# StavrosOrf/PoweFlowNet

Measured on AMD Instinct MI355X. Metric: graphs/sec fwd+bwd (train step incl. AdamW), case118v2 batch=128, higher is better.
Workload: dtype f32; 1 GPU; case118v2 (118 buses, 186 branches, synthetic topology) MaskEmbdMultiMPN standard.json (H129 L4 K3 dropout 0.2) training step fwd+MSELoss+bwd+AdamW, fp32; graphs_per_gpu=128, global_batch=128, nodes_per_gpu=15104, directed_edges_per_gpu=47616, parallelism=dp1, launch=hipGraph replay: one graph, undirected_on_device=True

## Files before the change

### poweflownet_amd/csrc/gemm_nt.hip

```cpp
#include <stddef.h>
#include <stdlib.h>
#include <string.h>

#include <algorithm>
#include <type_traits>
#include <vector>

#include "pfn_internal.hpp"

namespace pfn {

constexpr int NT_THREADS = 512;
constexpr int NT_WAVES = NT_THREADS / 64;
constexpr int NCH = 17;
constexpr int KP = 8 * NCH;
constexpr int NT_MAX_PIECES = 16;
constexpr int NT_LDS_BYTES = 160 * 1024;

__global__ __launch_bounds__(256) void pack_weights_kernel(const PackArgs a) {
    if (a.rng_advance && blockIdx.x == 0 && blockIdx.y == 0 && threadIdx.x == 0) a.rng_advance[1] += 1;
    if (a.stamp && blockIdx.x == 0 && blockIdx.y == 0 && threadIdx.x == 0) *a.stamp = a.stamp_value;
    if (a.mask_count > 0) {
        const int64_t nthr = (int64_t)gridDim.x * gridDim.y * blockDim.x;
        for (int64_t i = ((int64_t)blockIdx.y * gridDim.x + blockIdx.x) * blockDim.x + threadIdx.x; i < a.mask_count; i += nthr)
// ... 140 lines not shown
                case 1: wait_a<NCH - 2 + XW>(a_cur[m]); break;
                case 2: wait_a<NCH - 3 + XW>(a_cur[m]); break;
                default: wait_a<NCH - 4 + XW>(a_cur[m]); break;
            }
            const f32x4 av = a_cur[m];
#pragma unroll
            for (int i = 0; i < ((FAST && m == NFAST - 1) ? LS : 4); ++i) {
#pragma unroll
                for (int ct = 0; ct < CT; ++ct) acc[ct] = __builtin_amdgcn_mfma_f32_32x32x2f32(av[i], b[ct][i], acc[ct], 0, 0, 0);
#pragma unroll
                for (int c = 0; c < NR; ++c) racc[c] = fmaf(av[i], r[c][i], racc[c]);
            }
            slice(m);
            if (SLICED) {
#pragma unroll
                for (int c = 0; c < NR; ++c) PFN_OPAQUE(racc[c]);
            }
        }
        if ((m & 3) == 3 || m == NCH - 1) {
#pragma unroll
            for (int mm = m & ~3; mm <= m; ++mm) {
                if (FAST && DIET && mm < NFAST - 1) {
                    vload_x4(a_cur[mm], nbase + (size_t)mm * 8u * nkscale, vlane0);
                } else {
                    const uint32_t kk = min(kh4 + 8u * mm, (uint32_t)nkmax);
                    vload_x4(a_cur[mm], nbase, nvoff + nkscale * kk);
                }
            }
        }
        __builtin_amdgcn_sched_barrier(0);
    }
}

template <int CT, int VAR, bool PAIR = false, bool ILF = false>
__global__ __launch_bounds__(NT_THREADS, 1) void gemm_nt_kernel(const NtArgs a) {
    extern __shared__ __attribute__((aligned(16))) float lds[];
    constexpr int CTE = CT > 0 ? CT : 1;
    const int tid = threadIdx.x, lane = tid & 63;
    const int wave = __builtin_amdgcn_readfirstlane(tid >> 6);
    const int r32 = lane & 31, kh = lane >> 5;
    int bx = blockIdx.x, slice = blockIdx.y;
    {
        const int gx = gridDim.x, ns = gridDim.y, full = gx & ~7;
        const int lin = blockIdx.y * gx + blockIdx.x;
        if (ns > 1 && lin < full * ns) {
            const int chunk = lin / (8 * ns), r = lin - chunk * 8 * ns;
            slice = r >> 3;
            bx = chunk * 8 + (r & 7);
        } else if (ns > 1) {
            const int t = lin - full * ns, tail = gx - full;
            slice = t / tail;
            bx = full + (t - slice * tail);
        }
    }
    const int cg = wave & ((1 << a.cshift) - 1);
    const int rsub = wave >> a.cshift;
    const int rw = NT_WAVES >> a.cshift;
    const int tile0 = slice * a.tps + cg * CT;
    const bool mfma_on = CT > 0 && tile0 < a.nq;
    const bool rem_on = a.remv > 0 && slice == (int)gridDim.y - 1 && cg == 0;
    const int rem_col = 32 * a.nq;
    const int nrt = (a.M + 31) >> 5;
    const int rt_step = gridDim.x * rw;
    int rt = rsub * (int)gridDim.x + bx;

    auto prt = [&](int t) { return a.reverse ? nrt - 1 - t : t; };
    auto a_base = [&](int rt2, int p2) -> const char* {
        return reinterpret_cast<const char*>(a.piece[p2].A + (size_t)prt(rt2) * 32 * a.piece[p2].lda);
    };
// ... 68 lines not shown
    if constexpr (PAIR) {
#pragma unroll
        for (int ct = 0; ct < CTE; ++ct)
#pragma unroll
            for (int q = 0; q < 16; ++q) psum[ct][q] = 0.f;
    }
    f32x16 il_acc[ILF ? CTE : 1];
    float il_racc = 0.f, il_sc = 0.f, il_lo = 0.f;
    uint64_t il_ok[4] = {0ull, 0ull, 0ull, 0ull}, il_okr = 0ull;
    float* il_C = a.C[0];
    int il_rbase = 0;
    const int il_rs_ = a.c_cm_rows > 0 ? 4 : a.ldc, il_qs_ = a.c_cm_rows > 0 ? 32 * a.c_cm_rows : 32;
    const int il_rq_ = (rem_col >> 2) * (a.c_cm_rows > 0 ? 4 * a.c_cm_rows : 4);
    const uint32_t il_vc = (uint32_t)((r32 & 3) + 4 * kh) * (uint32_t)il_rs_ * 4u + (uint32_t)(r32 >> 2) * (a.c_cm_rows > 0 ? (uint32_t)a.c_cm_rows * 16u : 16u);
    const uint32_t il_vr = (uint32_t)r32 * (uint32_t)il_rs_ * 4u;
    if constexpr (ILF) {
#pragma unroll
        for (int ct = 0; ct < CTE; ++ct) {
#pragma unroll
            for (int q = 0; q < 16; ++q) il_acc[ct][q] = 0.f;
        }
        il_lo = a.act == ACT_RELU ? 0.f : __builtin_nanf("");
    }
    const int nr = rem_on ? (a.nrem > 1 ? 4 : 1) : 0;
    const float* extra = a.gate ? a.gate : a.resid;
    const int ldx = a.gate ? a.ldg : a.ldr;
    uint32_t kh4 = 4u * kh;
    auto rounds = [&](auto nfast_c, auto nr_c, auto ls_c) {
    constexpr int NFAST = decltype(nfast_c)::value, NR = decltype(nr_c)::value, LS = decltype(ls_c)::value;
    int p = 0;
    typedef const NtPiece __attribute__((address_space(4)))* NtPieceK;
    const NtPieceK pk = (NtPieceK)((const char __attribute__((address_space(4)))*)__builtin_amdgcn_kernarg_segment_ptr() + offsetof(NtArgs, piece));
    int cur_gl = pk[0].gl, cur_lds = pk[0].lds_off, cur_klen = pk[0].klen;
    while (true) {
        PFN_OPAQUE(kh4);
        int np = p + 1, nrt_ = rt;
        if (np == a.npiece) {
            np = 0;
            nrt_ = rt + rt_step;
        }
        const bool more = nrt_ < nrt;
        const int group = cur_gl & 255;
        const bool flush_after = !more || (cur_gl >> 8) != 0;
        const int pi = more ? np : p;
        const NtPieceK nx = pk + pi;
        const float* nxA = nx->A;
        const int nx_lda = nx->lda, nx_kscale = nx->kscale, nkmax = nx->kmax, nx_klen = nx->klen, nx_gl = nx->gl, nx_lds = nx->lds_off;
        const int nrt2 = prt(more ? nrt_ : rt);
        const char* nbase = reinterpret_cast<const char*>(nxA + (size_t)nrt2 * 32 * nx_lda);
        const uint32_t nvoff = (uint32_t)(min(r32, a.M - 1 - nrt2 * 32) * nx_lda) * 4u;
        const int rbase = prt(rt) * 32;
        const int jrow = (r32 & 3) + 4 * kh, uc4 = r32 & ~3;
        const bool tile_full = rbase + 32 <= a.M;
        auto rowok = [&](int g) { return rbase + jrow + 8 * g < a.M; };
        auto colok = [&](int q) { return 32 * q + uc4 < a.ldc; };
        auto qfull = [&](int q) { return 32 * q + 32 <= a.ldc; };
        auto ubase = [&](int q, int g, int ld, int cm) -> size_t {
            return cm > 0 ? ((size_t)8 * q * cm + rbase + 8 * g) * 4 : (size_t)(rbase + 8 * g) * ld + 32 * q;
        };
        auto lane_off = [&](int ld, int cm) -> uint32_t {
            return cm > 0 ? ((uint32_t)(uc4 >> 2) * (uint32_t)cm + jrow) * 16u : ((uint32_t)jrow * (uint32_t)ld + uc4) * 4u;
        };
        f32x4 aux[CTE][4], raux;
        float il_rs = 0.f;
        if constexpr (ILF) {
            if (a.rowscale)
// ... 65 lines not shown
                } else {
                    il_sc = use_bias ? 1.f : 0.f;
                }
#pragma unroll
                for (int ct = 0; ct < CTE; ++ct)
#pragma unroll
                    for (int q = 0; q < 16; ++q) {
                        il_acc[ct][q] = acc[ct][q];
                        acc[ct][q] = 0.f;
                    }
                il_racc = racc[0];
                racc[0] = racc[1] = racc[2] = racc[3] = 0.f;
                il_C = a.C[group];
                il_rbase = rbase;
#pragma unroll
                for (int g = 0; g < 4; ++g) il_ok[g] = __ballot(rbase + jrow + 8 * g < a.M);
                il_okr = __ballot(rem_on && kh == 0 && rbase + r32 < a.M);
                if (!more) {
#pragma unroll
                    for (int u = 0; u < 4 * CT; ++u) {
                        il_unit(u);
                        __builtin_amdgcn_sched_barrier(0);
                    }
                    if (NR > 0) il_rem();
                    break;
                }
                p = np;
                rt = nrt_;
                cur_gl = nx_gl;
                cur_lds = nx_lds;
                cur_klen = nx_klen;
                continue;
            }
            nt_multiply<CT, NR, NFAST, LS>(acc, racc, a_cur, S, klen, a.tps, tsel, kh4, r32, nbase, nvoff, nkmax,
                                           (uint32_t)nx_kscale);
        }
        if (flush_after) {
            if (CT > 0) {
                if (CT == 2) PFN_XDL_SETTLE("+v"(acc[0]), "+v"(acc[CTE - 1]));
                else PFN_XDL_SETTLE("+v"(acc[0]));
            }
            if constexpr (PAIR) {
#pragma unroll
                for (int ct = 0; ct < CTE; ++ct)
#pragma unroll
                    for (int q = 0; q < 16; ++q) {
                        acc[ct][q] = psum[ct][q] + acc[ct][q];
                        psum[ct][q] = 0.f;
                    }
#pragma unroll
                for (int e = 0; e < 4; ++e) {
                    racc[e] = prsum[e] + racc[e];
                    prsum[e] = 0.f;
                }
            }
            float* C = a.C[group];
            const int gf = a.gflags[group];
            const bool use_bias = a.bias && (a.bias_group < 0 || a.bias_group == group);
            if (has_aux) {
                if (CT == 2)
                    asm volatile("s_waitcnt vmcnt(17)" : "+v"(aux[0][0]), "+v"(aux[0][1]), "+v"(aux[0][2]), "+v"(aux[0][3]),
                                 "+v"(aux[CTE - 1][0]), "+v"(aux[CTE - 1][1]), "+v"(aux[CTE - 1][2]), "+v"(aux[CTE - 1][3]), "+v"(raux));
                else
                    asm volatile("s_waitcnt vmcnt(17)" : "+v"(aux[0][0]), "+v"(aux[0][1]), "+v"(aux[0][2]), "+v"(aux[0][3]), "+v"(raux));
                if (a.rowscale) {
#pragma unroll
                    for (int g = 0; g < 4; ++g) {
                        const float rs = aux[0][g][0];
// ... 24 lines not shown
                    }
                    if (gf & 1) {
#pragma unroll
                        for (int g = 0; g < 4; ++g) {
                            const float4 old = *reinterpret_cast<const float4*>(dst_of(g));
                            v[g][0] += old.x; v[g][1] += old.y; v[g][2] += old.z; v[g][3] += old.w;
                        }
                    }
                    if (!raw) {
                        const f32x4 cb4 = *reinterpret_cast<const f32x4*>(lds + a.bias_lds_off + col0);
                        if (use_bias && !ep.has_rowscale) {
#pragma unroll
                            for (int g = 0; g < 4; ++g)
#pragma unroll
                                for (int e = 0; e < 4; ++e) v[g][e] += cb4[e];
                        }
                        if (ep.has_rowscale) {
#pragma unroll
                            for (int g = 0; g < 4; ++g)
#pragma unroll
                                for (int e = 0; e < 4; ++e) v[g][e] = fmaf(aux[ct][g][e], cb4[e], v[g][e]);
                        }
                        if (ep.has_resid) {
#pragma unroll
                            for (int g = 0; g < 4; ++g)
#pragma unroll
                                for (int e = 0; e < 4; ++e) v[g][e] += aux[ct][g][e];
                        }
                        if (ep.act == ACT_RELU) {
#pragma unroll
                            for (int g = 0; g < 4; ++g)
#pragma unroll
                                for (int e = 0; e < 4; ++e) v[g][e] = fmaxf(v[g][e], 0.f);
                        } else if (ep.act == ACT_DROPOUT_RELU) {
                            uint32_t cgv = (uint32_t)(col0 >> 2);
                            PFN_OPAQUE(cgv);
#pragma unroll
                            for (int g = 0; g < 4; ++g) {
                                float u[4];
                                dropout_uniform4(ep.dk, (uint32_t)(row_of(g) + a.row0), cgv, u);
#pragma unroll
                                for (int e = 0; e < 4; ++e) v[g][e] = (u[e] >= ep.p_drop && v[g][e] > 0.f) ? v[g][e] * ep.keep_scale : 0.f;
                            }
                        }
                        if (ep.has_gate) {
#pragma unroll
                            for (int g = 0; g < 4; ++g)
#pragma unroll
                                for (int e = 0; e < 4; ++e) v[g][e] = aux[ct][g][e] > 0.f ? v[g][e] * ep.gate_scale : 0.f;
                        }
                    }
                    {
                        const int q = tile0 + ct;
                        const uint32_t vc = lane_off(a.ldc, a.c_cm_rows);
                        const bool unmasked = tile_full && qfull(q);
#pragma unroll
                        for (int g = 0; g < 4; ++g) {
                            const char* cb = reinterpret_cast<const char*>(C + ubase(q, g, a.ldc, a.c_cm_rows));
                            if (unmasked || (rowok(g) && colok(q))) vstore_x4_sv<(CT < 2)>(cb, vc, f32x4{v[g][0], v[g][1], v[g][2], v[g][3]});
                        }
                    }
                }
            }
            if (rem_on) {
                float v[4];
#pragma unroll
                for (int e = 0; e < 4; ++e) v[e] = racc[e] + __shfl_xor(racc[e], 32);
                const int row = rbase + r32;
                if (kh == 0 && row < a.M) {
                    float* dst = C + act_off(row, rem_col, a.ldc, a.c_cm_rows);
                    if (gf & 1) {
                        const float4 old = *reinterpret_cast<const float4*>(dst);
                        v[0] += old.x; v[1] += old.y; v[2] += old.z; v[3] += old.w;
                    }
                    if (!raw) {
                        const f32x4 rcb = *reinterpret_cast<const f32x4*>(lds + a.bias_lds_off + rem_col);
                        float ud[4] = {1.f, 1.f, 1.f, 1.f};
                        if (ep.act == ACT_DROPOUT_RELU) {
                            uint32_t cgv = (uint32_t)(rem_col >> 2);
                            PFN_OPAQUE(cgv);
                            dropout_uniform4(ep.dk, (uint32_t)(row + a.row0), cgv, ud);
                        }
#pragma unroll
                        for (int e = 0; e < 4; ++e) {
                            float x = v[e] + ((use_bias && !ep.has_rowscale) ? rcb[e] : 0.f);
                            if (ep.has_rowscale) x = fmaf(raux[e], rcb[e], x);
                            if (ep.has_resid) x += raux[e];
                            if (ep.act == ACT_RELU) {
                                x = fmaxf(x, 0.f);
                            } else if (ep.act == ACT_DROPOUT_RELU) {
                                x = (ud[e] >= ep.p_drop && x > 0.f) ? x * ep.keep_scale : 0.f;
                            }
                            if (ep.has_gate) x = raux[e] > 0.f ? x * ep.gate_scale : 0.f;
                            v[e] = rem_col + e < ep.ncols ? x : 0.f;
                        }
                    }
                    vstore_x4<(CT < 2)>(dst, f32x4{v[0], v[1], v[2], v[3]});
                }
            }
#pragma unroll
            for (int ct = 0; ct < CTE; ++ct)
#pragma unroll
                for (int q = 0; q < 16; ++q) acc[ct][q] = 0.f;
            racc[0] = racc[1] = racc[2] = racc[3] = 0.f;
        }
        if constexpr (PAIR) {
            if (!flush_after) {
                if (CT > 0) PFN_XDL_SETTLE("+v"(acc[0]));
#pragma unroll
                for (int ct = 0; ct < CTE; ++ct)
#pragma unroll
                    for (int q = 0; q < 16; ++q) {
                        psum[ct][q] += acc[ct][q];
                        acc[ct][q] = 0.f;
                    }
#pragma unroll
                for (int e = 0; e < 4; ++e) {
                    prsum[e] += racc[e];
                    racc[e] = 0.f;
                }
            }
        }
// ... 330 lines not shown
    float* C = a.C[0];
    const float* cvec = a.rowscale ? a.rowbias : a.bias;
    const int col0 = 32 * q + (r32 & ~3);
#pragma unroll
    for (int g = 0; g < 4; ++g) {
        float t4[4] = {v16[4 * g], v16[4 * g + 1], v16[4 * g + 2], v16[4 * g + 3]};
        quad_transpose(t4, lane);
        const int row = rbase + (r32 & 3) + 8 * g + 4 * kh;
        if (row < a.M) {
            const float rs = a.rowscale ? a.rowscale[row] : 1.f;
            float o[4];
#pragma unroll
            for (int e = 0; e < 4; ++e) {
                const int col = col0 + e;
                float x = t4[e] + ((cvec && col < a.ncols) ? rs * cvec[col] : 0.f);
                if (a.act == ACT_RELU) x = fmaxf(x, 0.f);
                o[e] = col < a.ncols ? x : 0.f;
            }
            *reinterpret_cast<float4*>(C + act_off(row, col0, a.ldc, a.c_cm_rows)) = make_float4(o[0], o[1], o[2], o[3]);
        }
    }
    if (rem) {
        const float tot = rsum + __shfl_xor(rsum, 32);
        const int row = rbase + r32;
        if (kh == 0 && row < a.M) {
            const float rs = a.rowscale ? a.rowscale[row] : 1.f;
            float x = tot + (cvec ? rs * cvec[128] : 0.f);
            if (a.act == ACT_RELU) x = fmaxf(x, 0.f);
            *reinterpret_cast<float4*>(C + act_off(row, 128, a.ldc, a.c_cm_rows)) = make_float4(x, 0.f, 0.f, 0.f);
        }
    }
}

template <int CT, int VAR, bool PAIR = false, bool ILF = false>
static int launch_variant(const NtArgs& k, dim3 grid, size_t lds_bytes, hipStream_t s) {
    static std::atomic<uint64_t> lds_raised{0};
    PFN_TRY(ensure_dynamic_lds(reinterpret_cast<const void*>(gemm_nt_kernel<CT, VAR, PAIR, ILF>), NT_LDS_BYTES, lds_raised));
    gemm_nt_kernel<CT, VAR, PAIR, ILF><<<grid, NT_THREADS, lds_bytes, s>>>(k);
    PFN_CHECK_LAUNCH();
    return PFN_OK;
}
static int pick_variant(const NtArgs& k, int CT) {
    const int nr = k.remv > 0 ? (k.nrem > 1 ? 4 : 1) : 0;
    bool diet_ok = true;
    for (int i = 0; i < k.npiece; ++i) diet_ok = diet_ok && k.piece[i].kmax >= k.piece[i].klen - 12;
    if (k.kuni == KP && nr <= 1 && diet_ok) return k.klast == 1 ? 0 : 1;
    if (k.kuni == KP - 8 && nr == 0 && diet_ok) return 2;
    return CT < 2 ? 3 : -1;
}

static int launch_gemm_nt_rows(const GemmArgs& a, hipStream_t s, bool top);
int launch_gemm_nt(const GemmArgs& a, hipStream_t s) { return launch_gemm_nt_rows(a, s, true); }
static int launch_gemm_nt_rows(const GemmArgs& a, hipStream_t s, bool top) {
    if (a.M == 0) return PFN_OK;
    int remv, nq;
    col_plan(a.ldc, remv, nq);
    if (a.ldc % 4) {
        set_error("gemm_nt: output row stride %d must be a multiple of 4", a.ldc);
        return PFN_EINVAL;
    }
    if (a.bias && a.rowscale) {
        set_error("gemm_nt: a GEMM takes a bias or a row-scaled bias, not both");
        return PFN_EINVAL;
    }
    double flops = 0.0, bytes = (double)a.ngroup * a.M * a.ncols * 4.0;
    std::vector<NtPiece> pieces;
    std::vector<int> last_steps;
    for (int t = 0; t < a.nterm; ++t) {
        const GemmTerm& tm = a.term[t];
        if (tm.lda % 4 != 0 || tm.lda < ((tm.K + 3) & ~3)) {
            set_error("gemm_nt: operand row stride %d must be a multiple of 4 and >= roundup(K=%d, 4)", tm.lda, tm.K);
// ... 152 lines not shown
            pieces[i1].lds_off = (int)(used / sizeof(float));
            used += piece_bytes(pieces[i1], tps);
            ++i1;
        }
        if (i1 == i0) {
            set_error("gemm_nt: a %d-row weight piece does not fit in LDS", pieces[i0].klen);
            return PFN_EINVAL;
        }
        k.npiece = (int)(i1 - i0);
        k.bias_lds_off = (int)(used / sizeof(float));
        k.kuni = pieces[i0].klen;
        k.klast = 1;
        for (size_t i = i0; i < i1; ++i) {
            if (pieces[i].klen != k.kuni) k.kuni = 0;
            if (last_steps[i] != 1) k.klast = 4;
        }
        bool here[8] = {false, false, false, false, false, false, false, false};
        for (size_t i = i0; i < i1; ++i) {
            k.piece[i - i0] = pieces[i];
            k.piece[i - i0].gl = pieces[i].group | ((i + 1 == i1 || pieces[i + 1].group != pieces[i].group) ? 256 : 0);
            here[pieces[i].group] = true;
        }
        for (int g = 0; g < 8; ++g) {
            bool later = false;
            for (size_t i = i1; i < pieces.size(); ++i) later |= pieces[i].group == g;
            k.gflags[g] = (seen[g] ? 1 : 0) | (later ? 2 : 0);
            seen[g] |= here[g];
        }
        int rc = PFN_EINVAL;
        const int var = pick_variant(k, CT);
        const size_t lb = used + bias_bytes;
        static const bool no_pair = diag_env("PFN_NO_NT_PAIR") != nullptr;
        const bool pair = !no_pair && CT == 1 && (var == 0 || var == 1) && k.npiece >= 3;
        if (pair) rc = var == 0 ? launch_variant<1, 0, true>(k, grid, lb, s) : launch_variant<1, 1, true>(k, grid, lb, s);
        static const bool no_ilf = diag_env("PFN_NO_NT_ILF") != nullptr;
        bool ilf = !no_ilf && CT == 2 && var == 0 && !a.gate && !a.resid && (a.act == ACT_NONE || a.act == ACT_RELU) && tps % 2 == 0 &&
                   nq % tps == 0 && a.ldc == 32 * nq + (remv > 0 ? 4 : 0);
        for (int i = 0; i < k.npiece; ++i) ilf = ilf && (k.piece[i].gl >> 8) != 0;
        for (int g = 0; g < 8; ++g) ilf = ilf && k.gflags[g] == 0;
        if (ilf) rc = launch_variant<2, 0, false, true>(k, grid, lb, s);
#define PFN_NT_CASE(CT_, V_) if (!pair && !ilf && CT == CT_ && var == V_) rc = launch_variant<CT_, V_>(k, grid, lb, s)
        PFN_NT_CASE(0, 0); PFN_NT_CASE(0, 1); PFN_NT_CASE(0, 2); PFN_NT_CASE(0, 3);
        PFN_NT_CASE(1, 0); PFN_NT_CASE(1, 1); PFN_NT_CASE(1, 2); PFN_NT_CASE(1, 3);
        PFN_NT_CASE(2, 0); PFN_NT_CASE(2, 1); PFN_NT_CASE(2, 2);
#undef PFN_NT_CASE
        if (var < 0) set_error("gemm_nt: no CT = %d kernel for this launch (kuni %d, nrem %d)", CT, k.kuni, k.nrem);
        if (rc != PFN_OK) return rc;
        i0 = i1;
    }
    return PFN_OK;
}

}
```

### poweflownet_amd/csrc/graph.hip

```cpp
#include <atomic>
#include <stdarg.h>
#include <stdio.h>
#include <stdlib.h>

#include <algorithm>

#include "pfn_internal.hpp"

namespace pfn {

static thread_local char g_err[512] = "";
void set_error(const char* fmt, ...) {
    va_list ap;
    va_start(ap, fmt);
    vsnprintf(g_err, sizeof(g_err), fmt, ap);
    va_end(ap);
}
const char* last_error() { return g_err; }

const char* diag_env(const char* name) { return getenv(name); }
int next_sweep_direction() {
    static const bool off = diag_env("PFN_NO_SERPENTINE") != nullptr;
    static thread_local unsigned n = 0;
    return off ? 0 : (int)(n++ & 1u);
}

int device_cus() {
    static std::atomic<int> cus[64];
    int dev = 0;
    if (hipGetDevice(&dev) != hipSuccess) return 256;
    std::atomic<int>& slot = cus[dev & 63];
    int v = slot.load(std::memory_order_relaxed);
    if (v == 0) {
        hipDeviceProp_t prop;
        v = (hipGetDeviceProperties(&prop, dev) == hipSuccess && prop.multiProcessorCount > 0) ? prop.multiProcessorCount : 256;
        slot.store(v, std::memory_order_relaxed);
    }
    return v;
}

int ensure_dynamic_lds(const void* kernel, int bytes, std::atomic<uint64_t>& done) {
    int dev = 0;
    PFN_CHECK_HIP(hipGetDevice(&dev));
    const uint64_t bit = 1ull << (dev & 63);
    if (done.load(std::memory_order_acquire) & bit) return PFN_OK;
    PFN_CHECK_HIP(hipFuncSetAttribute(kernel, hipFuncAttributeMaxDynamicSharedMemorySize, bytes));
    done.fetch_or(bit, std::memory_order_release);
    return PFN_OK;
}

GraphView graph_view(void* ws, int64_t n, int64_t e) {
    Carver c(ws);
    GraphView g;
// ... 408 lines not shown
```

### poweflownet_amd/csrc/pfn_internal.hpp

```cpp
#pragma once
#include <hip/hip_runtime.h>
#include <stddef.h>
#include <stdint.h>

#include <atomic>

#include "../../include/pfn_hip.h"
#include "device_prims.hpp"

namespace pfn {

void set_error(const char* fmt, ...);
#define PFN_CHECK_ARG(cond, ...)                 \
    do {                                         \
        if (!(cond)) {                           \
            ::pfn::set_error(__VA_ARGS__);       \
            return PFN_EINVAL;                   \
        }                                        \
    } while (0)
#define PFN_CHECK_HIP(expr)                                                              \
    do {                                                                                 \
        hipError_t e__ = (expr);                                                         \
        if (e__ != hipSuccess) {                                                         \
            ::pfn::set_error("%s failed: %s (%s:%d)", #expr, hipGetErrorString(e__), __FILE__, __LINE__); \
// ... 310 lines not shown
    const float* ea_out;
    const float* w1;
    float* dP;
    float* dQ;
    float* dWe_partial;
    int ldgo, fo, ld, h, fi;
    struct MseTail mse;
    const unsigned* gates = nullptr;
};
bool ea_seg_fit(int seg, int n, int fe, int ld, bool bwd);
bool front_seg_fit(int seg, int n, int h, int fe);
int launch_front_seg_fwd(const GraphView& g, const struct FrontFwdArgs& f, const PackJob* jobs, int njobs, uint64_t* rng_advance,
                         const SlotEa* slot_ea, int* stamp, int stamp_value, const float* ea, float* S, int seg, hipStream_t s);
int ea_seg_blocks(int seg, int n, int ld);
int launch_ea_seg_fwd(const GraphView& g, const EaSegFwdArgs& a, int seg, hipStream_t s);
int launch_ea_seg_bwd(const GraphView& g, const EaSegBwdArgs& a, int seg, hipStream_t s);

struct SegLinHopsArgs {
    const float* A0;
    const float* A1;
    const float* B0;
    const float* B1;
    const float* rowscale;
    const float* rowbias;
    const float* gate;
    const uint64_t* rng;
    float* y;
    float* xk;
    size_t stride;
    float gate_scale, p_drop;
    uint32_t rng_stream;
    int act, lda, K, ld, ncols, ldg, nhops;
    int adjt;
};
bool seg_lin_hops_fit(int seg, int n, int ld, int K, int ncols, int nhops, int nterm);
int launch_seg_lin_hops(const GraphView& g, const SegLinHopsArgs& a, int seg, hipStream_t s);


struct EdgeBwdArgs {
    const float* P;
    const float* Q;
    const float* dS;
    const float* edge_attr;
    const float* w1;
    float* dP;
    float* dQ;
    float* dWe_partial;
    float* grad_edge_attr;
    int ld, h, fi, fe;
    const float* gout = nullptr;
    const float* w2 = nullptr;
    int fo = 0;
    const unsigned* mask = nullptr;
    float* gea_tmp = nullptr;
};
int edge_bwd_dst_blocks(const GraphView& g, int ld);
int launch_edge_bwd(const GraphView& g, const EdgeBwdArgs& a, const int64_t* edge_index_unused, hipStream_t s);
int launch_edge_attr_grad(const GraphView& g, const EdgeBwdArgs& a, hipStream_t s);
struct DweJob {
    const float* partial;
    float* gw1;
    int nblocks, ldw, col0, pad_;
};
constexpr int DWE_MAX_JOBS = 16;
struct DweJobs { DweJob job[DWE_MAX_JOBS]; };
template <int LANES>
// ... 50 lines not shown
    const float* x;
    const void* mask;
    const float *wa, *ba, *wb, *bb, *w1, *b1;
    float *maskf, *me_h, *x0, *P, *Q;
    int* mask_counts = nullptr;
    unsigned* gates = nullptr;
};
int launch_front_fwd_pack(const FrontFwdArgs& f, const PackJob* jobs, int njobs, uint64_t* rng_advance, hipStream_t s,
                          const SlotEa* slot_ea = nullptr, int* stamp = nullptr, int stamp_value = 0);
int launch_front_bwd(int n, int h, int ldw1, const float* dP, const float* dQ, const float* me_h, const float* w1,
                     const float* wb, float* g0, float* dh, hipStream_t s);
size_t front_bwd_wg_scratch_floats(int n, int h);
int launch_front_bwd_wg(int n, int h, int ldw1, const float* dP, const float* dQ, const float* maskf, const float* w1, const float* wa,
                        const float* ba, const float* wb, float* g0, float* scratch, float* gwa, float* gba, float* gwb, float* gbb,
                        hipStream_t s, const int* stamp = nullptr, int stamp_want = 0);
int launch_front_meh(int n, int h, const void* mask, int mask_dtype, const float* wa, const float* ba, float* me_h, hipStream_t s);
int launch_front_pq(int n, int h, int ldw1, const float* x0, const float* w1, const float* b1, float* P, float* Q, hipStream_t s);

int launch_pad_rows(const float* src, int64_t ld_src, float* dst, int64_t ld_dst, int64_t rows, int64_t f,
                    hipStream_t s);
int launch_export_edge_gates(const GraphView& g, const float* P, const float* Q, const float* ea, const float* w1, int ld, int h, int fi,
                             int fe, uint8_t* out, hipStream_t s);
int launch_export_row_gates(int64_t n, int h, int ld, const float* y, int cm, uint8_t* out, hipStream_t s);

struct DropKey { uint32_t k0, k1, stream, off; };
__host__ __device__ __forceinline__ DropKey drop_key(uint64_t seed, uint64_t offset, uint32_t stream) {
    DropKey k;
    k.k0 = (uint32_t)seed;
    k.k1 = (uint32_t)(seed >> 32) ^ (uint32_t)(offset >> 32);
    k.stream = stream;
    k.off = (uint32_t)offset;
    return k;
}
__device__ __forceinline__ void philox4x32_10(uint32_t (&c)[4], uint32_t k0, uint32_t k1) {
#pragma unroll
    for (int r = 0; r < 10; ++r) {
        const uint64_t p0 = (uint64_t)0xD2511F53u * c[0], p1 = (uint64_t)0xCD9E8D57u * c[2];
        const uint32_t hi0 = (uint32_t)(p0 >> 32), lo0 = (uint32_t)p0;
        const uint32_t hi1 = (uint32_t)(p1 >> 32), lo1 = (uint32_t)p1;
        c[0] = hi1 ^ c[1] ^ k0;
        c[1] = lo1;
        c[2] = hi0 ^ c[3] ^ k1;
        c[3] = lo0;
        k0 += 0x9E3779B9u;
        k1 += 0xBB67AE85u;
    }
}
__device__ __forceinline__ void dropout_uniform4(const DropKey& k, uint32_t row, uint32_t cg, float (&u)[4]) {
    uint32_t c[4] = {row, cg, k.stream, k.off};
    philox4x32_10(c, k.k0, k.k1);
#pragma unroll
    for (int i = 0; i < 4; ++i) u[i] = (float)(c[i] >> 8) * (1.0f / 16777216.0f);
}

}
```

### poweflownet_amd/csrc/seg_lin_hops.hip

```cpp
#include <stdlib.h>

#include <algorithm>

#include "pfn_internal.hpp"
#include "seg_tile.hpp"

namespace pfn {

constexpr int SLH_REM_FLOATS = SG_NCH * 32;

struct SlhLds {
    float* t0;
    float* t1;
    float* B[2];
    float* R[2];
    float* bias;
    float* dinv;
    float* rsc;
    float* rq;
    int* rp;
    int* nb;
};
__host__ __device__ inline size_t slh_union_floats(int trows, int nterm) {
    const size_t tile = (size_t)trows * SG_TW, img = (size_t)nterm * SG_NCH * 256;
// ... 92 lines not shown
    if (tid < SG_TW) {
        const int col = seg_col_of_tile(sc, tid);
        bv = (a.rowbias && col >= 0 && col < a.ncols) ? a.rowbias[col] : 0.f;
    }
    const int nitems = rows * sc.cw;
    float4 gv[3];
#pragma unroll
    for (int j = 0; j < 3; ++j) {
        const int it = tid + j * SG_THREADS;
        gv[j] = make_float4(1.f, 1.f, 1.f, 1.f);
        if (a.gate && it < nitems) {
            const int lr = it / sc.cw, lc = it - lr * sc.cw;
            gv[j] = ld4(a.gate + (size_t)(r0 + lr) * a.ldg + seg_gcol(sc, lc));
        }
    }
    const int nbv = (nb_in_lds && tid < ne) ? nbr[e0 + tid] : 0;
    if (tid <= rows) l.rp[tid] = rpv - e0;
    if (tid < rows) {
        l.dinv[tid] = dv;
        l.rsc[tid] = rsv;
    }
    if (nb_in_lds && tid < ne) l.nb[tid] = nbv - r0;
    if (tid < SG_TW) l.bias[tid] = bv;
    if (sc.rem && tid < SLH_REM_FLOATS / 4) {
        st4(l.R[0] + tid * 4, rem0);
        if (NTERM > 1) st4(l.R[1] + tid * 4, rem1);
    }
    unsigned gbits = 0u;
#pragma unroll
    for (int j = 0; j < 3; ++j)
        gbits |= ((gv[j].x > 0.f ? 1u : 0u) | (gv[j].y > 0.f ? 2u : 0u) | (gv[j].z > 0.f ? 4u : 0u) | (gv[j].w > 0.f ? 8u : 0u)) << (4 * j);
    seg_drain_visible();
    if (mfma_on) seg_load_a_async(ta, (NTERM > 1 && mterm) ? a.A1 : a.A0, a.lda, r0 + 32 * mtile, r0 + rows - 1, lane);
    lds_barrier();
    for (int term = 0; term < NTERM; ++term) {
        if (mfma_on && mterm == term) {
            f32x16 acc;
            float racc = 0.f;
            if (term == 0) {
#pragma unroll
                for (int j = 0; j < 16; ++j) acc[j] = 0.f;
            } else {
                slh_load_tile(acc, l.t0, 32 * mtile, lane);
                if (sc.rem) racc = l.rq[mtile * 64 + lane];
            }
            if (sc.rem) slh_mma<1, true, true>(acc, racc, ta, l.B[term], l.R[term], lane);
            else slh_mma<1, false, true>(acc, racc, ta, l.B[term], l.R[term], lane);
            seg_store_tile(acc, sc.q, nullptr, a.ncols, l.t0, 32 * mtile, lane);
            if (sc.rem) {
                if (term + 1 < NTERM) {
                    l.rq[mtile * 64 + lane] = racc;
                } else {
                    const float tot = racc + __shfl_xor(racc, 32);
                    if (lane < 32) st4(l.t0 + (size_t)(32 * mtile + lane) * SG_TW + 32, make_float4(tot, 0.f, 0.f, 0.f));
                }
            }
        }
        __syncthreads();
    }
    DropKey dk = DropKey{0u, 0u, 0u, 0u};
    float keep_scale = 1.f;
    if (a.act == ACT_DROPOUT_RELU) {
        dk = drop_key(a.rng[0], a.rng[1], a.rng_stream);
        keep_scale = 1.0f / (1.0f - a.p_drop);
    }
#pragma unroll
    for (int j = 0; j < 3; ++j) {
        const int it = tid + j * SG_THREADS;
        if (it < nitems) {
            const int lr = it / sc.cw, lc = it - lr * sc.cw;
            const int tc = seg_tcol(sc, lc), gc = seg_gcol(sc, lc);
            const float4 v4 = ld4(l.t0 + (size_t)lr * SG_TW + tc);
            float v[4] = {v4.x, v4.y, v4.z, v4.w};
            if (a.rowscale) {
                const float rs = l.rsc[lr];
                const float4 cb = ld4(l.bias + tc);
                v[0] = fmaf(rs, cb.x, v[0]); v[1] = fmaf(rs, cb.y, v[1]); v[2] = fmaf(rs, cb.z, v[2]); v[3] = fmaf(rs, cb.w, v[3]);
            }
            if (a.act == ACT_RELU) {
#pragma unroll
                for (int e = 0; e < 4; ++e) v[e] = fmaxf(v[e], 0.f);
            } else if (a.act == ACT_DROPOUT_RELU) {
                float u[4];
                dropout_uniform4(dk, (uint32_t)(r0 + lr), (uint32_t)(gc >> 2), u);
#pragma unroll
                for (int e = 0; e < 4; ++e) v[e] = (u[e] >= a.p_drop && v[e] > 0.f) ? v[e] * keep_scale : 0.f;
            }
            if (a.gate) {
#pragma unroll
                for (int e = 0; e < 4; ++e) v[e] = ((gbits >> (4 * j + e)) & 1u) ? v[e] * a.gate_scale : 0.f;
            }
#pragma unroll
            for (int e = 0; e < 4; ++e) v[e] = gc + e < a.ncols ? v[e] : 0.f;
            const float4 o4 = make_float4(v[0], v[1], v[2], v[3]);
            st4(l.t0 + (size_t)lr * SG_TW + tc, o4);
            st4_wt(a.y + (size_t)(r0 + lr) * a.ld + gc, o4);
        }
    }
    lds_barrier();
    uint32_t cur = 0, nxt = (uint32_t)(trows * SG_TW);
    auto walk_item = [&](int it, float* gout, bool last) {
        const int lr = it / sc.cw, lc = it - lr * sc.cw;
        const int tc = seg_tcol(sc, lc), gc = seg_gcol(sc, lc);
        const float di = l.dinv[lr];
        const int beg = l.rp[lr], end = l.rp[lr + 1], lastp = end - 1;
        float4 h = make_float4(0.f, 0.f, 0.f, 0.f);
        for (int p = beg; p < end; p += 4) {
            int s_[4];
#pragma unroll
            for (int u = 0; u < 4; ++u) s_[u] = nb_in_lds ? l.nb[min(p + u, lastp)] : nbr[e0 + min(p + u, lastp)] - r0;
            float w_[4];
            float4 x_[4];
#pragma unroll
            for (int u = 0; u < 4; ++u) {
// ... 91 lines not shown
    if (seg <= 0 || seg > SG_MAX_ROWS || n <= 0 || n % seg != 0) return false;
    const int gpb = std::max(1, SG_MAX_ROWS / seg);
    p.rows_pb = gpb * seg;
    p.trows = (p.rows_pb + 31) / 32 * 32;
    p.cap = std::min(p.rows_pb * 4, SG_THREADS);
    p.nblocks = (n + p.rows_pb - 1) / p.rows_pb;
    int remv, nq;
    col_plan(ld, remv, nq);
    p.ny = nq;
    return p.ny >= 1 && slh_lds_bytes(p.trows, p.rows_pb, p.cap, nterm) <= (size_t)SG_LDS_BYTES;
}

bool seg_lin_hops_fit(int seg, int n, int ld, int K, int ncols, int nhops, int nterm) {
    static const bool off = diag_env("PFN_NO_SEG_LIN_HOPS") != nullptr;
    const long per_cu = 4L;
    SlhPlan p;
    int remv, nq;
    col_plan(ld, remv, nq);
    return !off && nhops > 0 && nterm >= 1 && nterm <= 2 && ((K + 7) & ~7) == 8 * SG_NCH && K - (8 * SG_NCH - 8) == 1 &&
           ncols <= ld && ld == ld_of(ncols) && remv == 4 && ncols - 32 * nq == 1 && fused_hops_fit(seg, ld, n) &&
           slh_plan(seg, n, ld, nterm, p) && (long)p.nblocks * p.ny <= per_cu * device_cus();
}

int launch_seg_lin_hops(const GraphView& g, const SegLinHopsArgs& a, int seg, hipStream_t s) {
    const int nterm = a.A1 ? 2 : 1;
    SlhPlan p;
    if (!slh_plan(seg, g.n, a.ld, nterm, p)) {
        set_error("seg_lin_hops: %d-row graphs do not fit", seg);
        return PFN_EINVAL;
    }
    const size_t lds = slh_lds_bytes(p.trows, p.rows_pb, p.cap, nterm);
    const int* rp = a.adjt ? g.rowptr_out : g.rowptr_in;
    const int* nb = a.adjt ? g.out_dst : g.in_src;
    static std::atomic<uint64_t> raised1{0}, raised2{0};
    ProfScope ps(a.adjt ? "seg_lin_hops_bwd" : "seg_lin_hops_fwd", 0.0, 2.0 * g.n * (double)a.K * a.ncols * nterm, s);
    if (nterm == 1) {
        PFN_TRY(ensure_dynamic_lds(reinterpret_cast<const void*>(seg_lin_hops_kernel<1>), SG_LDS_BYTES, raised1));
        seg_lin_hops_kernel<1><<<dim3(p.nblocks, p.ny), SG_THREADS, lds, s>>>(g.n, p.rows_pb, p.trows, p.cap, rp, nb, g.dinv, a);
    } else {
        PFN_TRY(ensure_dynamic_lds(reinterpret_cast<const void*>(seg_lin_hops_kernel<2>), SG_LDS_BYTES, raised2));
        seg_lin_hops_kernel<2><<<dim3(p.nblocks, p.ny), SG_THREADS, lds, s>>>(g.n, p.rows_pb, p.trows, p.cap, rp, nb, g.dinv, a);
    }
    PFN_CHECK_LAUNCH();
    return PFN_OK;
}

}
```

Before: 221,000 graphs/s.

## Draw dropout Philox bits early, interleaved with MFMA rounds and before barriers

Splits the Philox 10-round generator into resumable slices. The paired NT GEMM kernel now computes dropout keep-bits in small chunks interleaved with its matrix multiply pieces, and the seg_lin_hops kernel computes them before the LDS barrier and hop loop. The epilogue then applies precomputed bitmasks instead of running the full RNG serially after accumulation. This hides RNG ALU latency under memory and MFMA work, at the cost of extra live registers and a restricted set of eligible launch configurations.

```diff
diff --git a/poweflownet_amd/csrc/gemm_nt.hip b/poweflownet_amd/csrc/gemm_nt.hip
--- a/poweflownet_amd/csrc/gemm_nt.hip
+++ b/poweflownet_amd/csrc/gemm_nt.hip
@@ -196,9 +196,10 @@
     }
 }
 
-template <int CT, int VAR, bool PAIR = false, bool ILF = false>
+template <int CT, int VAR, bool PAIR = false, bool ILF = false, bool EDR = false>
 __global__ __launch_bounds__(NT_THREADS, 1) void gemm_nt_kernel(const NtArgs a) {
     extern __shared__ __attribute__((aligned(16))) float lds[];
+    static_assert(!EDR || (CT == 1 && !ILF), "the early dropout draw exists at one quarter per wave");
     constexpr int CTE = CT > 0 ? CT : 1;
     const int tid = threadIdx.x, lane = tid & 63;
     const int wave = __builtin_amdgcn_readfirstlane(tid >> 6);
@@ -333,6 +334,7 @@
     typedef const NtPiece __attribute__((address_space(4)))* NtPieceK;
     const NtPieceK pk = (NtPieceK)((const char __attribute__((address_space(4)))*)__builtin_amdgcn_kernarg_segment_ptr() + offsetof(NtArgs, piece));
     int cur_gl = pk[0].gl, cur_lds = pk[0].lds_off, cur_klen = pk[0].klen;
+    uint32_t ebits = 0u;
     while (true) {
         PFN_OPAQUE(kh4);
         int np = p + 1, nrt_ = rt;
@@ -464,8 +466,31 @@
                 cur_klen = nx_klen;
                 continue;
             }
-            nt_multiply<CT, NR, NFAST, LS>(acc, racc, a_cur, S, klen, a.tps, tsel, kh4, r32, nbase, nvoff, nkmax,
-                                           (uint32_t)nx_kscale);
+            if constexpr (EDR) {
+                const int dg = p & 3;
+                const uint32_t dsh = 4u * (uint32_t)dg;
+                const uint32_t drow = (uint32_t)(rbase + jrow + 8 * dg + a.row0), rrow = (uint32_t)(rbase + r32 + a.row0);
+                uint32_t cgv = (uint32_t)((32 * tile0 + uc4) >> 2), rcgv = (uint32_t)(rem_col >> 2);
+                PFN_OPAQUE(cgv);
+                PFN_OPAQUE(rcgv);
+                DropDraw dt;
+                auto slice = [&](int m) {
+                    const int d = m / 5, j = m - 5 * d;
+                    if (d < 1 + (NR > 0 ? 1 : 0)) {
+                        if (j == 0) drop_draw_begin(dt, ep.dk, d ? rrow : drow, d ? rcgv : cgv);
+                        drop_draw_rounds(dt, ep.dk, 2 * j, 2 * j + 2);
+                        if (j == 4) {
+                            const uint32_t kb = drop_draw_bits(dt, ep.p_drop);
+                            ebits = d ? (ebits & 0xFFFFu) | (kb << 16) : (ebits & ~(0xFu << dsh)) | (kb << dsh);
+                        }
+                    }
+                };
+                nt_multiply<CT, NR, NFAST, LS, 0, true>(acc, racc, a_cur, S, klen, a.tps, tsel, kh4, r32, nbase, nvoff, nkmax,
+                                                        (uint32_t)nx_kscale, slice);
+            } else {
+                nt_multiply<CT, NR, NFAST, LS>(acc, racc, a_cur, S, klen, a.tps, tsel, kh4, r32, nbase, nvoff, nkmax,
+                                               (uint32_t)nx_kscale);
+            }
         }
         if (flush_after) {
             if (CT > 0) {
@@ -556,6 +581,12 @@
                             for (int g = 0; g < 4; ++g)
 #pragma unroll
                                 for (int e = 0; e < 4; ++e) v[g][e] = fmaxf(v[g][e], 0.f);
+                        } else if (EDR && ep.act == ACT_DROPOUT_RELU) {
+#pragma unroll
+                            for (int g = 0; g < 4; ++g)
+#pragma unroll
+                                for (int e = 0; e < 4; ++e)
+                                    v[g][e] = (((ebits >> (4 * g + e)) & 1u) && v[g][e] > 0.f) ? v[g][e] * ep.keep_scale : 0.f;
                         } else if (ep.act == ACT_DROPOUT_RELU) {
                             uint32_t cgv = (uint32_t)(col0 >> 2);
                             PFN_OPAQUE(cgv);
@@ -600,7 +631,7 @@
                     if (!raw) {
                         const f32x4 rcb = *reinterpret_cast<const f32x4*>(lds + a.bias_lds_off + rem_col);
                         float ud[4] = {1.f, 1.f, 1.f, 1.f};
-                        if (ep.act == ACT_DROPOUT_RELU) {
+                        if (!EDR && ep.act == ACT_DROPOUT_RELU) {
                             uint32_t cgv = (uint32_t)(rem_col >> 2);
                             PFN_OPAQUE(cgv);
                             dropout_uniform4(ep.dk, (uint32_t)(row + a.row0), cgv, ud);
@@ -612,6 +643,8 @@
                             if (ep.has_resid) x += raux[e];
                             if (ep.act == ACT_RELU) {
                                 x = fmaxf(x, 0.f);
+                            } else if (EDR && ep.act == ACT_DROPOUT_RELU) {
+                                x = (((ebits >> (16 + e)) & 1u) && x > 0.f) ? x * ep.keep_scale : 0.f;
                             } else if (ep.act == ACT_DROPOUT_RELU) {
                                 x = (ud[e] >= ep.p_drop && x > 0.f) ? x * ep.keep_scale : 0.f;
                             }
@@ -1008,11 +1041,11 @@
     }
 }
 
-template <int CT, int VAR, bool PAIR = false, bool ILF = false>
+template <int CT, int VAR, bool PAIR = false, bool ILF = false, bool EDR = false>
 static int launch_variant(const NtArgs& k, dim3 grid, size_t lds_bytes, hipStream_t s) {
     static std::atomic<uint64_t> lds_raised{0};
-    PFN_TRY(ensure_dynamic_lds(reinterpret_cast<const void*>(gemm_nt_kernel<CT, VAR, PAIR, ILF>), NT_LDS_BYTES, lds_raised));
-    gemm_nt_kernel<CT, VAR, PAIR, ILF><<<grid, NT_THREADS, lds_bytes, s>>>(k);
+    PFN_TRY(ensure_dynamic_lds(reinterpret_cast<const void*>(gemm_nt_kernel<CT, VAR, PAIR, ILF, EDR>), NT_LDS_BYTES, lds_raised));
+    gemm_nt_kernel<CT, VAR, PAIR, ILF, EDR><<<grid, NT_THREADS, lds_bytes, s>>>(k);
     PFN_CHECK_LAUNCH();
     return PFN_OK;
 }
@@ -1231,7 +1264,11 @@
         const size_t lb = used + bias_bytes;
         static const bool no_pair = diag_env("PFN_NO_NT_PAIR") != nullptr;
         const bool pair = !no_pair && CT == 1 && (var == 0 || var == 1) && k.npiece >= 3;
-        if (pair) rc = var == 0 ? launch_variant<1, 0, true>(k, grid, lb, s) : launch_variant<1, 1, true>(k, grid, lb, s);
+        bool edr = pair && a.act == ACT_DROPOUT_RELU && early_dropout_on() && k.npiece >= 4;
+        for (int i = 0; i < k.npiece; ++i) edr = edr && k.piece[i].group == k.piece[0].group && ((k.piece[i].gl >> 8) != 0) == (i + 1 == k.npiece);
+        for (int g = 0; g < 8; ++g) edr = edr && k.gflags[g] == 0;
+        if (pair && edr) rc = var == 0 ? launch_variant<1, 0, true, false, true>(k, grid, lb, s) : launch_variant<1, 1, true, false, true>(k, grid, lb, s);
+        else if (pair) rc = var == 0 ? launch_variant<1, 0, true>(k, grid, lb, s) : launch_variant<1, 1, true>(k, grid, lb, s);
         static const bool no_ilf = diag_env("PFN_NO_NT_ILF") != nullptr;
         bool ilf = !no_ilf && CT == 2 && var == 0 && !a.gate && !a.resid && (a.act == ACT_NONE || a.act == ACT_RELU) && tps % 2 == 0 &&
                    nq % tps == 0 && a.ldc == 32 * nq + (remv > 0 ? 4 : 0);
diff --git a/poweflownet_amd/csrc/graph.hip b/poweflownet_amd/csrc/graph.hip
--- a/poweflownet_amd/csrc/graph.hip
+++ b/poweflownet_amd/csrc/graph.hip
@@ -19,6 +19,10 @@
 const char* last_error() { return g_err; }
 
 const char* diag_env(const char* name) { return getenv(name); }
+bool early_dropout_on() {
+    static const bool off = diag_env("PFN_NO_EARLY_DROPOUT") != nullptr;
+    return !off;
+}
 int next_sweep_direction() {
     static const bool off = diag_env("PFN_NO_SERPENTINE") != nullptr;
     static thread_local unsigned n = 0;
diff --git a/poweflownet_amd/csrc/pfn_internal.hpp b/poweflownet_amd/csrc/pfn_internal.hpp
--- a/poweflownet_amd/csrc/pfn_internal.hpp
+++ b/poweflownet_amd/csrc/pfn_internal.hpp
@@ -366,6 +366,7 @@
     uint32_t rng_stream;
     int act, lda, K, ld, ncols, ldg, nhops;
     int adjt;
+    int early_drop = 0;
 };
 bool seg_lin_hops_fit(int seg, int n, int ld, int K, int ncols, int nhops, int nterm);
 int launch_seg_lin_hops(const GraphView& g, const SegLinHopsArgs& a, int seg, hipStream_t s);
@@ -482,25 +483,42 @@
     k.off = (uint32_t)offset;
     return k;
 }
-__device__ __forceinline__ void philox4x32_10(uint32_t (&c)[4], uint32_t k0, uint32_t k1) {
+__device__ __forceinline__ void philox4x32_rounds(uint32_t (&c)[4], uint32_t k0, uint32_t k1, int r0, int r1) {
 #pragma unroll
-    for (int r = 0; r < 10; ++r) {
+    for (int r = r0; r < r1; ++r) {
         const uint64_t p0 = (uint64_t)0xD2511F53u * c[0], p1 = (uint64_t)0xCD9E8D57u * c[2];
         const uint32_t hi0 = (uint32_t)(p0 >> 32), lo0 = (uint32_t)p0;
         const uint32_t hi1 = (uint32_t)(p1 >> 32), lo1 = (uint32_t)p1;
-        c[0] = hi1 ^ c[1] ^ k0;
+        c[0] = hi1 ^ c[1] ^ (k0 + (uint32_t)r * 0x9E3779B9u);
         c[1] = lo1;
-        c[2] = hi0 ^ c[3] ^ k1;
+        c[2] = hi0 ^ c[3] ^ (k1 + (uint32_t)r * 0xBB67AE85u);
         c[3] = lo0;
-        k0 += 0x9E3779B9u;
-        k1 += 0xBB67AE85u;
-    }
-}
+    }
+}
+__device__ __forceinline__ void philox4x32_10(uint32_t (&c)[4], uint32_t k0, uint32_t k1) { philox4x32_rounds(c, k0, k1, 0, 10); }
 __device__ __forceinline__ void dropout_uniform4(const DropKey& k, uint32_t row, uint32_t cg, float (&u)[4]) {
     uint32_t c[4] = {row, cg, k.stream, k.off};
     philox4x32_10(c, k.k0, k.k1);
 #pragma unroll
     for (int i = 0; i < 4; ++i) u[i] = (float)(c[i] >> 8) * (1.0f / 16777216.0f);
 }
-
-}
+struct DropDraw { uint32_t c[4]; };
+__device__ __forceinline__ void drop_draw_begin(DropDraw& d, const DropKey& k, uint32_t row, uint32_t cg) {
+    d.c[0] = row; d.c[1] = cg; d.c[2] = k.stream; d.c[3] = k.off;
+}
+__device__ __forceinline__ void drop_draw_rounds(DropDraw& d, const DropKey& k, int r0, int r1) { philox4x32_rounds(d.c, k.k0, k.k1, r0, r1); }
+__device__ __forceinline__ uint32_t drop_draw_bits(const DropDraw& d, float p_drop) {
+    uint32_t bits = 0u;
+#pragma unroll
+    for (int i = 0; i < 4; ++i) bits |= ((float)(d.c[i] >> 8) * (1.0f / 16777216.0f) >= p_drop ? 1u : 0u) << i;
+    return bits;
+}
+__device__ __forceinline__ uint32_t dropout_keep4(const DropKey& k, uint32_t row, uint32_t cg, float p_drop) {
+    DropDraw d;
+    drop_draw_begin(d, k, row, cg);
+    drop_draw_rounds(d, k, 0, 10);
+    return drop_draw_bits(d, p_drop);
+}
+bool early_dropout_on();
+
+}
diff --git a/poweflownet_amd/csrc/seg_lin_hops.hip b/poweflownet_amd/csrc/seg_lin_hops.hip
--- a/poweflownet_amd/csrc/seg_lin_hops.hip
+++ b/poweflownet_amd/csrc/seg_lin_hops.hip
@@ -148,6 +148,21 @@
         gbits |= ((gv[j].x > 0.f ? 1u : 0u) | (gv[j].y > 0.f ? 2u : 0u) | (gv[j].z > 0.f ? 4u : 0u) | (gv[j].w > 0.f ? 8u : 0u)) << (4 * j);
     seg_drain_visible();
     if (mfma_on) seg_load_a_async(ta, (NTERM > 1 && mterm) ? a.A1 : a.A0, a.lda, r0 + 32 * mtile, r0 + rows - 1, lane);
+    const bool early = NTERM == 1 && a.early_drop;
+    unsigned dbits = 0u;
+    if constexpr (NTERM == 1) {
+        if (early) {
+            const DropKey dk0 = drop_key(a.rng[0], a.rng[1], a.rng_stream);
+#pragma unroll
+            for (int j = 0; j < 3; ++j) {
+                const int it = tid + j * SG_THREADS;
+                if (it < nitems) {
+                    const int lr = it / sc.cw, lc = it - lr * sc.cw;
+                    dbits |= dropout_keep4(dk0, (uint32_t)(r0 + lr), (uint32_t)(seg_gcol(sc, lc) >> 2), a.p_drop) << (4 * j);
+                }
+            }
+        }
+    }
     lds_barrier();
     for (int term = 0; term < NTERM; ++term) {
         if (mfma_on && mterm == term) {
@@ -196,6 +211,9 @@
             if (a.act == ACT_RELU) {
 #pragma unroll
                 for (int e = 0; e < 4; ++e) v[e] = fmaxf(v[e], 0.f);
+            } else if (a.act == ACT_DROPOUT_RELU && early) {
+#pragma unroll
+                for (int e = 0; e < 4; ++e) v[e] = (((dbits >> (4 * j + e)) & 1u) && v[e] > 0.f) ? v[e] * keep_scale : 0.f;
             } else if (a.act == ACT_DROPOUT_RELU) {
                 float u[4];
                 dropout_uniform4(dk, (uint32_t)(r0 + lr), (uint32_t)(gc >> 2), u);
@@ -353,14 +371,16 @@
     const size_t lds = slh_lds_bytes(p.trows, p.rows_pb, p.cap, nterm);
     const int* rp = a.adjt ? g.rowptr_out : g.rowptr_in;
     const int* nb = a.adjt ? g.out_dst : g.in_src;
+    SegLinHopsArgs ka = a;
+    ka.early_drop = nterm == 1 && a.act == ACT_DROPOUT_RELU && early_dropout_on();
     static std::atomic<uint64_t> raised1{0}, raised2{0};
     ProfScope ps(a.adjt ? "seg_lin_hops_bwd" : "seg_lin_hops_fwd", 0.0, 2.0 * g.n * (double)a.K * a.ncols * nterm, s);
     if (nterm == 1) {
         PFN_TRY(ensure_dynamic_lds(reinterpret_cast<const void*>(seg_lin_hops_kernel<1>), SG_LDS_BYTES, raised1));
-        seg_lin_hops_kernel<1><<<dim3(p.nblocks, p.ny), SG_THREADS, lds, s>>>(g.n, p.rows_pb, p.trows, p.cap, rp, nb, g.dinv, a);
+        seg_lin_hops_kernel<1><<<dim3(p.nblocks, p.ny), SG_THREADS, lds, s>>>(g.n, p.rows_pb, p.trows, p.cap, rp, nb, g.dinv, ka);
     } else {
         PFN_TRY(ensure_dynamic_lds(reinterpret_cast<const void*>(seg_lin_hops_kernel<2>), SG_LDS_BYTES, raised2));
-        seg_lin_hops_kernel<2><<<dim3(p.nblocks, p.ny), SG_THREADS, lds, s>>>(g.n, p.rows_pb, p.trows, p.cap, rp, nb, g.dinv, a);
+        seg_lin_hops_kernel<2><<<dim3(p.nblocks, p.ny), SG_THREADS, lds, s>>>(g.n, p.rows_pb, p.trows, p.cap, rp, nb, g.dinv, ka);
     }
     PFN_CHECK_LAUNCH();
     return PFN_OK;
```

Result: no change. 219,800 graphs/s (-0.5%).
